# fegennari/3DWorld

Hardware: NVIDIA H100
Metric: height cells/s @8192^2 8-octave domain-warp (higher is better)
Workload: dtype f32

## Files before the change

3dworld_b200/csrc/tw_heightgen.cu:

```cuda
#include "tw_internal.h"
#include <unordered_map>
#include <vector>
#include <algorithm>
#include "tw_noise.cuh"
#include "tw_noise2.cuh"
#include <stdlib.h>

namespace {

constexpr int F_TABLE = TW_F_TABLE_SIZE;

__device__ __forceinline__ float sinf_lut(const float *__restrict__ tab, float v) {
	return (v < 0.0f) ? -__ldg(tab + (tw_x86_f2i(TW_SSCALE*(-v))&(TW_TSIZE-1))) : __ldg(tab + (tw_x86_f2i(TW_SSCALE*v)&(TW_TSIZE-1)));
}
__device__ __forceinline__ float cosf_lut(const float *__restrict__ tab, float v) {
	return __ldg(tab + TW_TSIZE + (tw_x86_f2i(TW_SSCALE*fabsf(v))&(TW_TSIZE-1)));
}
__device__ __forceinline__ float smin(float a, float b) {return (b < a) ? b : a;}
__device__ __forceinline__ float smax(float a, float b) {return (a < b) ? b : a;}

struct PostParams {
	tw_hmap_params h;
	int   shape;
	int   need_postproc;
	int   enable_glaciate;
	int   glaciate;
	float zmax_est, zmax_est2, zmax_est2_inv, custom_exp;
	int   sine_on;
	float sm_scale, sm_freq, sine_offset;
	int   volcano_on;
	float volcano_freq;
	float mesh_scale_z_inv;
	float mdx, mdy, dx_inv, dy_inv;
	const unsigned *tile_perm;
	unsigned ngroups;
	unsigned skip_x0, skip_y0, skip_w, skip_h;
};

__device__ __forceinline__ float postproc_noise_zval(float z, const tw_hmap_params &h) {
	if (z > h.plat_bot) {z = h.plat_bot + h.plat_h*(z - h.plat_bot) + smin(h.plat_max, h.plat_s*(z - h.plat_bot));}
	if (z > h.crat_h  ) {z = h.crat_h - h.crat_s*(z - h.crat_h);}
	if (z > h.crack_lo && z < h.crack_hi) {z -= h.crack_d*smin(z - h.crack_lo, h.crack_hi - z);}
	return z;
}

__device__ __forceinline__ float volcano_height(float xi, float yi, const PostParams &P, const float *__restrict__ tab) {
	float const x = P.volcano_freq*xi, y = P.volcano_freq*yi, dist = __fsqrt_rn(x*x + y*y);
	if ((double)dist > 2.0) return 0.0f;
	float const val = cosf_lut(tab, x)*cosf_lut(tab, y);
	double const hd = 400.0*((double)val - 0.999);
	float const hole = (float)((0.0 < hd) ? hd : 0.0);
	float const peak = (float)(0.08*(double)val/(double)smax(0.04f, dist));
	return P.h.volcano_height*smax(0.0f, (peak - hole))*P.mesh_scale_z_inv;
}

__device__ __forceinline__ float glaciate_and_bias(float z, float smx, float smy, float cx, float cy, const PostParams &P, const float *__restrict__ tab) {
	if (!P.enable_glaciate) return z;
	if (P.glaciate) {
		float const relh = (z + P.zmax_est)*P.zmax_est2_inv;
		float const g = (P.custom_exp == 0.0f) ? relh*relh*relh : powf(relh, P.custom_exp);
		z = g*P.zmax_est2 - P.zmax_est;
	}
	if (P.sine_on) {
		z += smx*smy + P.sine_offset;
		if (P.volcano_on) {z += volcano_height(cx, cy, P, tab);}
	}
	return z;
}

__device__ __forceinline__ void block_minmax(float vmin, float vmax, unsigned *mm) {
	for (int o = 16; o > 0; o >>= 1) {
		vmin = fminf(vmin, __shfl_xor_sync(0xffffffffu, vmin, o));
		vmax = fmaxf(vmax, __shfl_xor_sync(0xffffffffu, vmax, o));
	}
	__shared__ float s_min[32], s_max[32];
	int const tid = threadIdx.x + blockDim.x*(threadIdx.y + blockDim.y*threadIdx.z);
	int const nw = (blockDim.x*blockDim.y*blockDim.z + 31) >> 5, w = tid >> 5, l = tid & 31;
	if (l == 0) {s_min[w] = vmin; s_max[w] = vmax;}
	__syncthreads();
	if (w == 0) {
		vmin = (l < nw) ? s_min[l] :  INFINITY;
		vmax = (l < nw) ? s_max[l] : -INFINITY;
		for (int o = 16; o > 0; o >>= 1) {
			vmin = fminf(vmin, __shfl_xor_sync(0xffffffffu, vmin, o));
			vmax = fmaxf(vmax, __shfl_xor_sync(0xffffffffu, vmax, o));
		}
		if (l == 0) {atomicMin(mm, tw_f2ord(vmin)); atomicMax(mm + 1, tw_f2ord(vmax));}
	}
}

struct NoiseParams {
	int   octaves;
	int   gen_shape;
	float4 oct[9];
	float xy_scale;
	float hmap_scale;
	float freq_last, rsum_last;
};

template<bool SIMPLEX, int SHAPE>
__device__ __forceinline__ float gen_noise(float xv, float yv, const NoiseParams &N) {
	float zval = 0.0f;
#pragma unroll 1
	for (int i = 0; i < N.octaves; ++i) {
		float4 const o = N.oct[i];
		float const px = o.x*xv + o.y, py = o.x*yv + o.z;
		float noise = SIMPLEX ? twn::simplex2(px, py) : twn::perlin2(px, py);
		if (SHAPE == 1) {noise = (float)((double)fabsf(noise) - 0.40);}
		if (SHAPE == 2) {noise = (float)(0.45 - (double)fabsf(noise));}
		zval = __fmaf_rn(o.w, noise, zval);
	}
	return zval;
}

template<bool SIMPLEX, bool WARP, int SHAPE>
__device__ __forceinline__ float get_noise_zval(float xval, float yval, const NoiseParams &N, const PostParams &P) {
	float xv = N.xy_scale*xval, yv = N.xy_scale*yval;
	if (WARP) {
		float const scale = 0.2f;
		float const dx1 = gen_noise<SIMPLEX, SHAPE>((float)((double)xv + 0.0), (float)((double)yv + 0.0), N);
		float const dy1 = gen_noise<SIMPLEX, SHAPE>((float)((double)xv + 5.2), (float)((double)yv + 1.3), N);
		float const wx = xv + scale*dx1, wy = yv + scale*dy1;
		float const dx2 = gen_noise<SIMPLEX, SHAPE>((float)((double)wx + 1.7), (float)((double)wy + 9.2), N);
		float const dy2 = gen_noise<SIMPLEX, SHAPE>((float)((double)wx + 8.3), (float)((double)wy + 2.8), N);
		xv += scale*dx2; yv += scale*dy2;
	}
	float z = gen_noise<SIMPLEX, SHAPE>(xv, yv, N);
	if (P.need_postproc) {z = postproc_noise_zval(z, P.h);}
	return z*N.hmap_scale;
}

template<bool SIMPLEX, bool WARP, int SHAPE>
__global__ void __launch_bounds__(256)
noise_grid_kernel(float *__restrict__ out, unsigned nx, unsigned ny, unsigned y_off, float mx0_single, float my0_single, const float2 *__restrict__ tile_origins,
	NoiseParams N, PostParams P, const float *__restrict__ sin_tab, unsigned *__restrict__ mm)
{
	unsigned const x = blockIdx.x*blockDim.x + threadIdx.x, y = y_off + blockIdx.y*blockDim.y + threadIdx.y, tile = blockIdx.z;
	float mx0 = mx0_single, my0 = my0_single;
	if (tile_origins) {float2 const o = __ldg(tile_origins + tile); mx0 = o.x; my0 = o.y;}
	float z = 0.0f;
	bool const valid = (x < nx && y < ny);
	if (valid) {
		float const xval = ((float)x*P.mdx + mx0)*P.dx_inv, yval = ((float)y*P.mdy + my0)*P.dy_inv;
		z = get_noise_zval<SIMPLEX, WARP, SHAPE>(xval, yval, N, P);
		float smx = 0.0f, smy = 0.0f;
		if (P.enable_glaciate && P.sine_on) {
			smx = P.sm_scale*cosf_lut(sin_tab, ((float)x*P.mdx + mx0)*P.dx_inv*P.sm_freq);
			smy = cosf_lut(sin_tab, ((float)y*P.mdy + my0)*P.dy_inv*P.sm_freq);
		}
		z = glaciate_and_bias(z, smx, smy, xval, yval, P, sin_tab);
		out[(size_t)tile*nx*ny + (size_t)y*nx + x] = z;
	}
	if (mm) {block_minmax(valid ? z : INFINITY, valid ? z : -INFINITY, mm + 2*tile);}
}

#ifndef TW_NOISE2_MIN_BLOCKS
#define TW_NOISE2_MIN_BLOCKS 2
#endif
#ifndef TW_NOISE2_PERSISTENT
#define TW_NOISE2_PERSISTENT 1
#endif
#ifndef TW_NOISE2_THREADS
#define TW_NOISE2_THREADS 512
#endif
#ifndef TW_NOISE2_BLOCK_CELLS
#define TW_NOISE2_BLOCK_CELLS 2048
#endif
static_assert(TW_NOISE2_BLOCK_CELLS % (2*TW_NOISE2_THREADS) == 0, "a block walks whole chunks of 2 cells per thread");
__device__ __forceinline__ bool noise_lattice_in_range(float2 xv, float2 yv, const NoiseParams &N) {
	float const bx = (fabsf(xv.x) + fabsf(yv.x))*N.freq_last + N.rsum_last, by = (fabsf(xv.y) + fabsf(yv.y))*N.freq_last + N.rsum_last;
	return (bx < 2097152.0f && by < 2097152.0f);
}

template<bool SIMPLEX, bool WARP> __host__ __device__ constexpr bool noise2_hash() {return SIMPLEX && WARP && TW_SIMPLEX_HASH_TABLE;}
template<bool HASH> __host__ __device__ constexpr int lut_entries() {return twn2::SIMPLEX_LUT_N + (HASH ? twn2::SIMPLEX_HASH_N : 0);}
template<bool HASH> __host__ __device__ constexpr int lut_slots() {return twn2::SIMPLEX_LUT_N*twn2::SIMPLEX_LUT_COPIES + (HASH ? twn2::SIMPLEX_HASH_N*twn2::SIMPLEX_HASH_COPIES : 0);}

template<bool SIMPLEX, int SHAPE, bool HASH>
__device__ __forceinline__ float2 noise2_octave(float2 xv, float2 yv, float4 o, unsigned L, float2 zval) {
	float2 const px = twn2::add2(twn2::mul2(xv, o.x), o.y), py = twn2::add2(twn2::mul2(yv, o.x), o.z);
	float2 noise = SIMPLEX ? ((TW_SIMPLEX_LUT > 0) ? twn2::simplex2_lut<HASH>(px, py, L) : twn2::simplex2(px, py)) : ((TW_SIMPLEX_LUT > 0) ? twn2::perlin2_lut(px, py, L) : twn2::perlin2(px, py));
	if (SHAPE == 1) {noise = make_float2((float)((double)fabsf(noise.x) - 0.40), (float)((double)fabsf(noise.y) - 0.40));}
	if (SHAPE == 2) {noise = make_float2((float)(0.45 - (double)fabsf(noise.x)), (float)(0.45 - (double)fabsf(noise.y)));}
	return twn2::fma2(noise, o.w, zval);
}

template<bool SIMPLEX, int SHAPE, bool HASH>
__device__ __forceinline__ float2 gen_noise2(float2 xv, float2 yv, const NoiseParams &N, unsigned L) {
	float2 zval = make_float2(0.0f, 0.0f);
	bool const in_range = noise_lattice_in_range(xv, yv, N);
	if (HASH && SHAPE == 0 && N.octaves == 8 && in_range) {
#pragma unroll
		for (int i = 0; i < 8; ++i) {zval = noise2_octave<SIMPLEX, SHAPE, HASH>(xv, yv, N.oct[i], L, zval);}
	}
	else if (in_range) {
#pragma unroll 1
		for (int i = 0; i < N.octaves; ++i) {zval = noise2_octave<SIMPLEX, SHAPE, HASH>(xv, yv, N.oct[i], L, zval);}
	}
	else {zval = make_float2(gen_noise<SIMPLEX, SHAPE>(xv.x, yv.x, N), gen_noise<SIMPLEX, SHAPE>(xv.y, yv.y, N));}
	return zval;
}

#ifndef TW_NOISE2_DUAL
#define TW_NOISE2_DUAL 0
#endif
template<bool SIMPLEX, int SHAPE, bool HASH>
__device__ __forceinline__ void gen_noise2_dual(float2 xa, float2 ya, float2 xb, float2 yb, const NoiseParams &N, unsigned L, float2 &za, float2 &zb) {
	if (TW_SIMPLEX_LUT > 0 && noise_lattice_in_range(xa, ya, N) && noise_lattice_in_range(xb, yb, N)) {
		float2 zva = make_float2(0.0f, 0.0f), zvb = make_float2(0.0f, 0.0f);
#pragma unroll 1
		for (int i = 0; i < N.octaves; ++i) {
			float4 const o = N.oct[i];
			float const f = o.x, rx = o.y, ry = o.z, mag = o.w;
			float2 const pxa = twn2::add2(twn2::mul2(xa, f), rx), pya = twn2::add2(twn2::mul2(ya, f), ry);
			float2 const pxb = twn2::add2(twn2::mul2(xb, f), rx), pyb = twn2::add2(twn2::mul2(yb, f), ry);
			float2 na = SIMPLEX ? twn2::simplex2_lut<HASH>(pxa, pya, L) : twn2::perlin2_lut(pxa, pya, L);
			float2 nb = SIMPLEX ? twn2::simplex2_lut<HASH>(pxb, pyb, L) : twn2::perlin2_lut(pxb, pyb, L);
			if (SHAPE == 1) {na = make_float2((float)((double)fabsf(na.x) - 0.40), (float)((double)fabsf(na.y) - 0.40)); nb = make_float2((float)((double)fabsf(nb.x) - 0.40), (float)((double)fabsf(nb.y) - 0.40));}
			if (SHAPE == 2) {na = make_float2((float)(0.45 - (double)fabsf(na.x)), (float)(0.45 - (double)fabsf(na.y))); nb = make_float2((float)(0.45 - (double)fabsf(nb.x)), (float)(0.45 - (double)fabsf(nb.y)));}
			zva = twn2::fma2(na, mag, zva); zvb = twn2::fma2(nb, mag, zvb);
		}
		za = zva; zb = zvb;
	}
	else {za = gen_noise2<SIMPLEX, SHAPE, HASH>(xa, ya, N, L); zb = gen_noise2<SIMPLEX, SHAPE, HASH>(xb, yb, N, L);}
}

__device__ __forceinline__ float dadd(float a, double b) {return (float)((double)a + b);}
__constant__ double2 warp_offsets[4] = {{0.0, 0.0}, {5.2, 1.3}, {1.7, 9.2}, {8.3, 2.8}};

template<bool SIMPLEX, bool WARP, int SHAPE>
__global__ void __launch_bounds__(TW_NOISE2_THREADS, TW_NOISE2_MIN_BLOCKS)
noise_grid2_kernel(float *__restrict__ out, unsigned nx, unsigned ny, unsigned y_off, unsigned y_end, float mx0_single, float my0_single, const float2 *__restrict__ tile_origins,
	NoiseParams N, PostParams P, const float *__restrict__ sin_tab, unsigned *__restrict__ mm, const float4 *__restrict__ simplex_lut)
{
	constexpr bool HASH = noise2_hash<SIMPLEX, WARP>();
	unsigned L = 0;
	if (TW_SIMPLEX_LUT > 0) {
		extern __shared__ float4 lut_s[];
		constexpr int G = twn2::SIMPLEX_LUT_N*twn2::SIMPLEX_LUT_COPIES;
		for (int e = threadIdx.x; e < lut_slots<HASH>(); e += blockDim.x) {
			lut_s[e] = __ldg(simplex_lut + ((e < G) ? e/twn2::SIMPLEX_LUT_COPIES : twn2::SIMPLEX_LUT_N + (e - G)/twn2::SIMPLEX_HASH_COPIES));
		}
		__syncthreads();
		L = twn2::simplex_lut_base(lut_s, threadIdx.x);
		asm volatile("" : "+r"(L) :: "memory");
	}
	unsigned const tile = blockIdx.z;
	float mx0 = mx0_single, my0 = my0_single;
	if (tile_origins) {float2 const o = __ldg(tile_origins + tile); mx0 = o.x; my0 = o.y;}
	size_t const c_end = (size_t)y_end*nx;
	float lo = INFINITY, hi = -INFINITY;
	constexpr unsigned NCH = TW_NOISE2_BLOCK_CELLS/(2*TW_NOISE2_THREADS);
#pragma unroll 1
	for (unsigned grp = blockIdx.x; grp < P.ngroups; grp += gridDim.x) {
#pragma unroll 1
	for (unsigned ch = 0; ch < NCH; ++ch) {
	size_t const c0 = (size_t)y_off*nx + 2*(((size_t)grp*NCH + ch)*blockDim.x + threadIdx.x);
	unsigned y, x;
	if (c_end <= 0xffffffffull) {unsigned const c32 = (unsigned)c0; y = c32/nx; x = c32 - y*nx;}
	else {y = (unsigned)(c0/nx); x = (unsigned)(c0 - (size_t)y*nx);}
	unsigned const xb = (x + 1 < nx) ? x + 1 : 0, yb = (x + 1 < nx) ? y : y + 1;
	bool const skip = (x - P.skip_x0 < P.skip_w && y - P.skip_y0 < P.skip_h && xb - P.skip_x0 < P.skip_w && yb - P.skip_y0 < P.skip_h);
	bool const valid0 = (c0 < c_end) && !skip, valid1 = (c0 + 1 < c_end) && !skip;
	float z0 = 0.0f, z1 = 0.0f;
	if (valid0) {
		using namespace twn2;
		float2 const xs = make_float2((float)x, (float)xb), ys = make_float2((float)y, (float)yb);
		float2 const xval = mul2(add2(mul2(xs, P.mdx), mx0), P.dx_inv);
		float2 const yval = mul2(add2(mul2(ys, P.mdy), my0), P.dy_inv);
		float2 xv = mul2(xval, N.xy_scale), yv = mul2(yval, N.xy_scale);
		float2 zz;
		if (WARP && !TW_NOISE2_DUAL) {
			float const scale = 0.2f;
			float2 bx = xv, by = yv, d = make_float2(0.0f, 0.0f);
#pragma unroll 1
			for (int s = 0; s < 5; ++s) {
				float2 sx = xv, sy = yv;
				if (s < 4) {double2 const o = warp_offsets[s]; sx = make_float2(dadd(bx.x, o.x), dadd(bx.y, o.x)); sy = make_float2(dadd(by.x, o.y), dadd(by.y, o.y));}
				float2 const r = gen_noise2<SIMPLEX, SHAPE, HASH>(sx, sy, N, L);
				if (s == 1) {bx = add2(xv, mul2(d, scale)); by = add2(yv, mul2(r, scale));}
				if (s == 3) {xv = add2(xv, mul2(d, scale)); yv = add2(yv, mul2(r, scale));}
				d = r;
			}
			zz = d;
		}
		else {
		if (WARP) {
			float const scale = 0.2f;
			float2 dx1, dy1, dx2, dy2;
			gen_noise2_dual<SIMPLEX, SHAPE, HASH>(make_float2(dadd(xv.x, 0.0), dadd(xv.y, 0.0)), make_float2(dadd(yv.x, 0.0), dadd(yv.y, 0.0)),
			                                      make_float2(dadd(xv.x, 5.2), dadd(xv.y, 5.2)), make_float2(dadd(yv.x, 1.3), dadd(yv.y, 1.3)), N, L, dx1, dy1);
			float2 const wx = add2(xv, mul2(dx1, scale)), wy = add2(yv, mul2(dy1, scale));
			gen_noise2_dual<SIMPLEX, SHAPE, HASH>(make_float2(dadd(wx.x, 1.7), dadd(wx.y, 1.7)), make_float2(dadd(wy.x, 9.2), dadd(wy.y, 9.2)),
			                                      make_float2(dadd(wx.x, 8.3), dadd(wx.y, 8.3)), make_float2(dadd(wy.x, 2.8), dadd(wy.y, 2.8)), N, L, dx2, dy2);
			xv = add2(xv, mul2(dx2, scale)); yv = add2(yv, mul2(dy2, scale));
		}
		zz = gen_noise2<SIMPLEX, SHAPE, HASH>(xv, yv, N, L);
		}
		z0 = zz.x; z1 = zz.y;
		if (P.need_postproc) {z0 = postproc_noise_zval(z0, P.h); z1 = postproc_noise_zval(z1, P.h);}
		z0 = z0*N.hmap_scale; z1 = z1*N.hmap_scale;
		float smx0 = 0.0f, smx1 = 0.0f, smy0 = 0.0f, smy1 = 0.0f;
		if (P.enable_glaciate && P.sine_on) {
			smx0 = P.sm_scale*cosf_lut(sin_tab, xval.x*P.sm_freq);
			smx1 = P.sm_scale*cosf_lut(sin_tab, xval.y*P.sm_freq);
			smy0 = cosf_lut(sin_tab, yval.x*P.sm_freq);
			smy1 = (yb == y) ? smy0 : cosf_lut(sin_tab, yval.y*P.sm_freq);
		}
		z0 = glaciate_and_bias(z0, smx0, smy0, xval.x, yval.x, P, sin_tab);
		z1 = glaciate_and_bias(z1, smx1, smy1, xval.y, yval.y, P, sin_tab);
		float *o = out + (size_t)(P.tile_perm ? __ldg(P.tile_perm + tile) : tile)*nx*ny + c0;
		if (valid1 && ((reinterpret_cast<size_t>(o) & 7) == 0)) {*reinterpret_cast<float2 *>(o) = make_float2(z0, z1);}
		else {o[0] = z0; if (valid1) {o[1] = z1;}}
	}
	lo = fminf(lo, fminf(valid0 ? z0 : INFINITY, valid1 ? z1 : INFINITY)); hi = fmaxf(hi, fmaxf(valid0 ? z0 : -INFINITY, valid1 ? z1 : -INFINITY));
	}
	}
	if (mm) {block_minmax(lo, hi, mm + 2*tile);}
}

template<bool SIMPLEX, bool WARP>
void launch_noise2(int shape, dim3 grid, dim3 block, cudaStream_t st, float *out, unsigned nx, unsigned ny, unsigned y_off, unsigned y_end, float mx0, float my0,
	const float2 *origins, const NoiseParams &N, const PostParams &P, const float *tab, unsigned *mm, const float4 *lut)
{
	size_t const lut_bytes = (TW_SIMPLEX_LUT > 0) ? (size_t)lut_slots<noise2_hash<SIMPLEX, WARP>()>()*sizeof(float4) : 0;
	if (lut_bytes > 48*1024) {
		switch (shape) {
		case 1:  cudaFuncSetAttribute(noise_grid2_kernel<SIMPLEX, WARP, 1>, cudaFuncAttributeMaxDynamicSharedMemorySize, (int)lut_bytes); break;
		case 2:  cudaFuncSetAttribute(noise_grid2_kernel<SIMPLEX, WARP, 2>, cudaFuncAttributeMaxDynamicSharedMemorySize, (int)lut_bytes); break;
		default: cudaFuncSetAttribute(noise_grid2_kernel<SIMPLEX, WARP, 0>, cudaFuncAttributeMaxDynamicSharedMemorySize, (int)lut_bytes); break;
		}
	}
	switch (shape) {
	case 1:  noise_grid2_kernel<SIMPLEX, WARP, 1><<<grid, block, lut_bytes, st>>>(out, nx, ny, y_off, y_end, mx0, my0, origins, N, P, tab, mm, lut); break;
	case 2:  noise_grid2_kernel<SIMPLEX, WARP, 2><<<grid, block, lut_bytes, st>>>(out, nx, ny, y_off, y_end, mx0, my0, origins, N, P, tab, mm, lut); break;
	default: noise_grid2_kernel<SIMPLEX, WARP, 0><<<grid, block, lut_bytes, st>>>(out, nx, ny, y_off, y_end, mx0, my0, origins, N, P, tab, mm, lut); break;
	}
}

constexpr int PERLIN_LUT_OFFSET = lut_entries<true>();
__global__ void simplex_lut_kernel(float4 *__restrict__ lut) {
	int const k = blockIdx.x*blockDim.x + threadIdx.x;
	if (k < twn2::SIMPLEX_LUT_N) {lut[k] = twn2::simplex_lut_entry((float)k); lut[PERLIN_LUT_OFFSET + k] = twn2::perlin_lut_entry((float)k);}
	if (k < twn2::SIMPLEX_HASH_N) {lut[twn2::SIMPLEX_LUT_N + k] = twn2::simplex_hash_entry((float)k);}
}
static int ensure_simplex_lut(tw_ctx *ctx) {
	if (ctx->d_simplex_lut) return TW_OK;
	static_assert(twn2::SIMPLEX_HASH_N <= twn2::SIMPLEX_LUT_N, "simplex_lut_kernel's grid covers the gradient tables");
	TW_CUDA(ctx, cudaMalloc(&ctx->d_simplex_lut, (PERLIN_LUT_OFFSET + twn2::SIMPLEX_LUT_N)*sizeof(float4)));
	simplex_lut_kernel<<<(twn2::SIMPLEX_LUT_N + 127)/128, 128, 0, ctx->stream>>>((float4 *)ctx->d_simplex_lut);
	TW_LAUNCH_CHECK(ctx);
	return TW_OK;
}

struct SineTabParams {
	float msx, msy, ms2, mesh_scale_z_inv;
	float dx, dy, mx0, my0;
	int   start;
	unsigned nx, ny, xpitch, ypitch;
	int   sine_on; float sm_scale, sm_freq, dx_inv, dy_inv;
};

__global__ void sine_tables_kernel(float *__restrict__ Xt, float *__restrict__ Yt, const float *__restrict__ T, const float *__restrict__ sin_tab, SineTabParams S,
	const float *__restrict__ origins = nullptr, unsigned nux = 0, size_t xstride = 0, size_t ystride = 0)
{
	unsigned const i = blockIdx.x*blockDim.x + threadIdx.x, k = blockIdx.y;
	bool const is_y = origins ? (blockIdx.z >= nux) : (blockIdx.z != 0);
	if (origins) {
		if (is_y) {S.my0 = __ldg(origins + blockIdx.z); Yt += (size_t)(blockIdx.z - nux)*ystride;}
		else      {S.mx0 = __ldg(origins + blockIdx.z); Xt += (size_t)blockIdx.z*xstride;}
	}
	unsigned const n = is_y ? S.ny : S.nx;
	if (i >= n) return;
	if (k == F_TABLE) {
		if (!S.sine_on) return;
		if (!is_y) {Xt[(size_t)k*S.xpitch + i] = S.sm_scale*cosf_lut(sin_tab, ((float)i*S.dx + S.mx0)*S.dx_inv*S.sm_freq);}
		else       {Yt[(size_t)k*S.ypitch + i] = cosf_lut(sin_tab, ((float)i*S.dy + S.my0)*S.dy_inv*S.sm_freq);}
		return;
	}
	if ((int)k < S.start) return;
	float const *s = T + 5*k;
	if (!is_y) {
		float const x_mult = S.msx*s[4];
		float const x_const = S.ms2*s[4] + s[2] + x_mult*S.mx0;
		float const xmdx = x_mult*S.dx;
		Xt[(size_t)k*S.xpitch + i] = sinf_lut(sin_tab, xmdx*(float)i + x_const);
	}
	else {
		float const y_mult = S.msy*s[3], y_scale = S.mesh_scale_z_inv*s[0];
		float const y_const = S.ms2*s[3] + s[1] + y_mult*S.my0;
		float const ymdy = y_mult*S.dy;
		Yt[(size_t)k*S.ypitch + i] = y_scale*sinf_lut(sin_tab, ymdy*(float)i + y_const);
	}
}

constexpr int ST = 64;
constexpr int SK = 45;

__global__ void __launch_bounds__(256)
sine_grid_kernel(float *__restrict__ out, unsigned nx, unsigned ny, const float *__restrict__ Xt, const float *__restrict__ Yt,
	unsigned xpitch, unsigned ypitch, int start_ix, PostParams P, float mx0, float my0, const float *__restrict__ sin_tab, unsigned *__restrict__ mm, unsigned y_off,
	const uint2 *__restrict__ tile_tabs = nullptr, const float2 *__restrict__ tile_origins = nullptr, size_t xstride = 0, size_t ystride = 0,
	const unsigned *__restrict__ tile_perm = nullptr)
{
	__shared__ float Xs[SK][ST], Ys[SK][ST];
	if (tile_tabs) {
		unsigned const tz = tile_perm ? __ldg(tile_perm + blockIdx.z) : blockIdx.z;
		uint2 const tt = __ldg(tile_tabs + tz);
		float2 const o = __ldg(tile_origins + tz);
		Xt += (size_t)tt.x*xstride; Yt += (size_t)tt.y*ystride; mx0 = o.x; my0 = o.y;
		out += (size_t)blockIdx.z*nx*ny;
		if (mm) {mm += 2*(size_t)blockIdx.z;}
	}
	unsigned const x_base = blockIdx.x*ST, y_base = y_off + blockIdx.y*ST;
	int const tid = threadIdx.x, tx = tid & 15, ty = tid >> 4;
	float2 acc2[4][2];
#pragma unroll
	for (int a = 0; a < 4; ++a) {acc2[a][0] = make_float2(0.0f, 0.0f); acc2[a][1] = make_float2(0.0f, 0.0f);}
	for (int k0 = start_ix; k0 < F_TABLE; k0 += SK) {
		int const kn = min(SK, F_TABLE - k0);
		__syncthreads();
		for (int e = tid; e < kn*ST; e += 256) {
			int const kk = e / ST, c = e % ST;
			unsigned const gx = x_base + c, gy = y_base + c;
			Xs[kk][c] = (gx < nx) ? __ldg(Xt + (size_t)(k0 + kk)*xpitch + gx) : 0.0f;
			Ys[kk][c] = (gy < ny) ? __ldg(Yt + (size_t)(k0 + kk)*ypitch + gy) : 0.0f;
		}
		__syncthreads();
#pragma unroll 5
		for (int kk = 0; kk < kn; ++kk) {
			float xv[4];
#pragma unroll
			for (int b = 0; b < 4; ++b) {xv[b] = Xs[kk][tx + 16*b];}
			float4 const yv4 = *reinterpret_cast<const float4 *>(&Ys[kk][ty*4]);
			float const yv[4] = {yv4.x, yv4.y, yv4.z, yv4.w};
			float2 const x01 = make_float2(xv[0], xv[1]), x23 = make_float2(xv[2], xv[3]);
#pragma unroll
			for (int a = 0; a < 4; ++a) {
				float2 const ya = twn2::splat(yv[a]);
				acc2[a][0] = twn2::add2(twn2::mul2(x01, ya), acc2[a][0]);
				acc2[a][1] = twn2::add2(twn2::mul2(x23, ya), acc2[a][1]);
			}
		}
	}
	float vmin = INFINITY, vmax = -INFINITY;
#pragma unroll
	for (int a = 0; a < 4; ++a) {
		unsigned const y = y_base + ty*4 + a;
		if (y >= ny) continue;
		float const smy = (P.enable_glaciate && P.sine_on) ? __ldg(Yt + (size_t)F_TABLE*ypitch + y) : 0.0f;
#pragma unroll
		for (int b = 0; b < 4; ++b) {
			unsigned const x = x_base + tx + 16*b;
			if (x >= nx) continue;
			float z = (b & 1) ? ((b >> 1) ? acc2[a][1].y : acc2[a][0].y) : ((b >> 1) ? acc2[a][1].x : acc2[a][0].x);
			if (P.shape == 1) {z = (float)((double)fabsf(z) - 2.0);}
			else if (P.shape == 2) {z = (float)(3.5 - (double)fabsf(z));}
			if (P.need_postproc) {z = postproc_noise_zval(z, P.h);}
			float const smx = (P.enable_glaciate && P.sine_on) ? __ldg(Xt + (size_t)F_TABLE*xpitch + x) : 0.0f;
			float cx = 0.0f, cy = 0.0f;
			if (P.volcano_on) {cx = ((float)x*P.mdx + mx0)*P.dx_inv; cy = ((float)y*P.mdy + my0)*P.dy_inv;}
			z = glaciate_and_bias(z, smx, smy, cx, cy, P, sin_tab);
			out[(size_t)y*nx + x] = z;
			vmin = fminf(vmin, z); vmax = fmaxf(vmax, z);
		}
	}
	if (mm) {block_minmax(vmin, vmax, mm);}
}

__global__ void init_minmax_kernel(unsigned *mm, uint32_t n) {
	uint32_t const i = blockIdx.x*blockDim.x + threadIdx.x;
	if (i < n) {mm[2*i] = 0xffffffffu; mm[2*i+1] = 0u;}
}

__global__ void minmax_kernel(const float *__restrict__ v, size_t n, unsigned *mm) {
	float vmin = INFINITY, vmax = -INFINITY;
	size_t const stride = (size_t)gridDim.x*blockDim.x;
	for (size_t i = (size_t)blockIdx.x*blockDim.x + threadIdx.x; i < n; i += stride) {float const z = __ldg(v + i); vmin = fminf(vmin, z); vmax = fmaxf(vmax, z);}
	block_minmax(vmin, vmax, mm);
}

__global__ void minmax_tiles_kernel(const float *__restrict__ v, size_t tile_elems, unsigned *mm, const unsigned *__restrict__ perm) {
	size_t const tile = perm ? __ldg(perm + blockIdx.x) : blockIdx.x;
	const float *t = v + tile*tile_elems;
	if (threadIdx.x == 0) {mm[2*tile] = 0xffffffffu; mm[2*tile + 1] = 0u;}
	__syncthreads();
	float vmin = INFINITY, vmax = -INFINITY;
	for (size_t i = threadIdx.x; i < tile_elems; i += blockDim.x) {float const z = __ldg(t + i); vmin = fminf(vmin, z); vmax = fmaxf(vmax, z);}
	block_minmax(vmin, vmax, mm + 2*tile);
}
__global__ void coarse_work_kernel(const float *__restrict__ coarse, unsigned cells, unsigned nt, float level, unsigned *__restrict__ work) {
	unsigned const t = blockIdx.x*blockDim.x + threadIdx.x;
	if (t >= nt) return;
	unsigned n = 0;
	for (unsigned i = 0; i < cells; ++i) {n += !(__ldg(coarse + (size_t)t*cells + i) < level);}
	work[t] = n;
}
__global__ void gather_origins_kernel(const float2 *__restrict__ org, const unsigned *__restrict__ order, unsigned nt, float2 *__restrict__ out) {
	unsigned const t = blockIdx.x*blockDim.x + threadIdx.x;
	if (t < nt) {out[t] = org[order[t]];}
}

template<bool SIMPLEX, bool WARP>
void launch_noise(int shape, dim3 grid, dim3 block, cudaStream_t st, float *out, unsigned nx, unsigned ny, unsigned y_off, float mx0, float my0,
	const float2 *origins, const NoiseParams &N, const PostParams &P, const float *tab, unsigned *mm)
{
	switch (shape) {
	case 1:  noise_grid_kernel<SIMPLEX, WARP, 1><<<grid, block, 0, st>>>(out, nx, ny, y_off, mx0, my0, origins, N, P, tab, mm); break;
	case 2:  noise_grid_kernel<SIMPLEX, WARP, 2><<<grid, block, 0, st>>>(out, nx, ny, y_off, mx0, my0, origins, N, P, tab, mm); break;
	default: noise_grid_kernel<SIMPLEX, WARP, 0><<<grid, block, 0, st>>>(out, nx, ny, y_off, mx0, my0, origins, N, P, tab, mm); break;
	}
}

}

int twi_init_minmax(tw_ctx *ctx, unsigned *d_mm_ord, uint32_t n) {
	init_minmax_kernel<<<(n + 255)/256, 256, 0, ctx->stream>>>(d_mm_ord, n);
	TW_LAUNCH_CHECK(ctx);
	return TW_OK;
}

int twi_minmax_tiles(tw_ctx *ctx, cudaStream_t st, const float *d_vals, size_t tile_elems, uint32_t nt, unsigned *d_mm_ord, const unsigned *d_perm) {
	minmax_tiles_kernel<<<nt, 256, 0, st>>>(d_vals, tile_elems, d_mm_ord, d_perm);
	TW_LAUNCH_CHECK(ctx);
	return TW_OK;
}
int twi_coarse_work(tw_ctx *ctx, const float *d_coarse, unsigned cells, uint32_t nt, float level, unsigned *d_work) {
	coarse_work_kernel<<<(nt + 127)/128, 128, 0, ctx->stream>>>(d_coarse, cells, nt, level, d_work);
	TW_LAUNCH_CHECK(ctx);
	return TW_OK;
}
int twi_gather_origins(tw_ctx *ctx, const void *d_org, const unsigned *d_order, uint32_t nt, void *d_out) {
	gather_origins_kernel<<<(nt + 255)/256, 256, 0, ctx->stream>>>((const float2 *)d_org, d_order, nt, (float2 *)d_out);
	TW_LAUNCH_CHECK(ctx);
	return TW_OK;
}

int twi_minmax(tw_ctx *ctx, const float *d_vals, size_t n, unsigned *d_mm_ord) {
	int const blocks = (int)((n + 255)/256 < ctx->num_sms*8 ? (n + 255)/256 : ctx->num_sms*8);
	minmax_kernel<<<blocks > 0 ? blocks : 1, 256, 0, ctx->stream>>>(d_vals, n, d_mm_ord);
	TW_LAUNCH_CHECK(ctx);
	return TW_OK;
}

static unsigned band_rows_for(tw_ctx *ctx, unsigned ny, unsigned nx, bool to_host) {
	if (!to_host || (size_t)nx*ny*sizeof(float) < ((size_t)32 << 20) || !ctx->aux_stream[0]) return ny;
	unsigned rows = ((ny + 15)/16 + 63) & ~63u;
	return rows < 64 ? 64 : rows;
}
static int band_join(tw_ctx *ctx) {
	cudaEvent_t ev;
	TW_CUDA(ctx, cudaEventCreateWithFlags(&ev, cudaEventDisableTiming));
	TW_CUDA(ctx, cudaEventRecord(ev, ctx->aux_stream[0]));
	TW_CUDA(ctx, cudaStreamWaitEvent(ctx->stream, ev, 0));
	TW_CUDA(ctx, cudaEventDestroy(ev));
	return TW_OK;
}

static int band_copy(tw_ctx *ctx, float *h_out, const float *d_out, unsigned nx, unsigned r0, unsigned r1) {
	cudaEvent_t ev;
	TW_CUDA(ctx, cudaEventCreateWithFlags(&ev, cudaEventDisableTiming));
	TW_CUDA(ctx, cudaEventRecord(ev, ctx->stream));
	TW_CUDA(ctx, cudaStreamWaitEvent(ctx->aux_stream[0], ev, 0));
	TW_CUDA(ctx, cudaEventDestroy(ev));
	TW_CUDA(ctx, cudaMemcpyAsync(h_out + (size_t)r0*nx, d_out + (size_t)r0*nx, (size_t)(r1 - r0)*nx*sizeof(float), cudaMemcpyDeviceToHost, ctx->aux_stream[0]));
	return TW_OK;
}

static PostParams make_post_params(const tw_height_params *p, int enable_glaciate, float dx, float dy) {
	PostParams P;
	memset(&P, 0, sizeof(P));
	P.h = p->hmap;
	P.shape = p->gen_shape;
	P.need_postproc = 1;
	P.enable_glaciate = (enable_glaciate != 0);
	P.glaciate = (p->glaciate != 0);
	P.zmax_est = p->zmax_est;
	P.zmax_est2 = (float)(2.0*p->zmax_est);
	P.zmax_est2_inv = (float)(1.0/P.zmax_est2);
	P.custom_exp = p->custom_glaciate_exp;
	P.sine_on = (p->hmap.sine_mag > 0.0f);
	P.sm_scale = p->hmap.sine_mag*p->mesh_scale_z_inv;
	P.sm_freq = p->mesh_scale*p->hmap.sine_freq;
	P.sine_offset = p->hmap.sine_bias*p->mesh_scale_z_inv;
	P.volcano_on = (p->hmap.volcano_width > 0.0f && p->hmap.volcano_height > 0.0f);
	P.volcano_freq = P.volcano_on ? p->mesh_scale/p->hmap.volcano_width : 0.0f;
	P.mesh_scale_z_inv = p->mesh_scale_z_inv;
	P.mdx = dx; P.mdy = dy; P.dx_inv = p->dx_val_inv; P.dy_inv = p->dy_val_inv;
	return P;
}

static bool make_noise_params(const tw_height_params *p, NoiseParams &N, bool &simplex) {
	memset(&N, 0, sizeof(N));
	int const start = p->start_eval_sin;
	if (start < 0 || start > F_TABLE) return false;
	N.octaves = 9 - start/10;
	N.gen_shape = p->gen_shape;
	float mag = 1.0f, freq = 1.0f, rx = p->rx, ry = p->ry;
	for (int i = 0; i < 9; ++i) {
		N.oct[i] = make_float4(freq, rx, ry, mag);
		mag *= 0.5f; freq *= 1.92f; rx *= 1.5f; ry *= 1.5f;
	}
	float4 const last = N.oct[N.octaves > 0 ? N.octaves - 1 : 0];
	N.freq_last = last.x; N.rsum_last = last.y + last.z;
	N.xy_scale = 0.0007f*p->mesh_scale;
	simplex = (p->gen_mode == TW_MGEN_SIMPLEX || p->gen_mode == TW_MGEN_SIMPLEX_GPU || p->gen_mode == TW_MGEN_DWARP_GPU);
	N.hmap_scale = (simplex ? 16.0f : 32.0f)*p->mesh_height*p->mesh_height_scale*p->mesh_scale_z_inv;
	return true;
}

int twi_heightgen(tw_ctx *ctx, const tw_grid2d *g, const tw_height_params *p, int enable_glaciate, int min_start_sin,
                  const float2 *d_tile_origins, uint32_t ntiles, float *d_out, unsigned *d_mm_ord, float *h_out_bands)
{
	unsigned const nx = g->nx, ny = g->ny;
	float const dx = g->dx, dy = g->dy;
	float const mx0 = dx*g->x0, my0 = dy*g->y0;
	if (ntiles == 0) ntiles = 1;

	PostParams P = make_post_params(p, enable_glaciate, dx, dy);
	P.skip_x0 = ctx->skip_rect[0]; P.skip_y0 = ctx->skip_rect[1]; P.skip_w = ctx->skip_rect[2]; P.skip_h = ctx->skip_rect[3];
	P.tile_perm = ctx->tile_perm;
	if (P.tile_perm && (p->gen_mode == TW_MGEN_SINE || getenv("TW_NOISE_SCALAR"))) return tw_set_error(ctx, TW_ERR_STATE, "internal: tile_perm is only wired into the paired noise kernels");

	if (p->gen_mode != TW_MGEN_SINE) {
		NoiseParams N;
		bool simplex = false;
		if (!make_noise_params(p, N, simplex)) return tw_set_error(ctx, TW_ERR_ARG, "start_eval_sin %d out of range", p->start_eval_sin);
		bool const warp = (p->gen_mode == TW_MGEN_DWARP_GPU);
		{int const rc = ensure_simplex_lut(ctx); if (rc) return rc;}
		const float4 *lut = (const float4 *)ctx->d_simplex_lut + (simplex ? 0 : PERLIN_LUT_OFFSET);
		unsigned const band_rows = band_rows_for(ctx, ny, nx, h_out_bands != nullptr && ntiles == 1);
		for (unsigned r0 = 0; r0 < ny; r0 += band_rows) {
			unsigned const r1 = (ny - r0 < band_rows) ? ny : r0 + band_rows;
			static bool const use_scalar = (getenv("TW_NOISE_SCALAR") != nullptr);
			if (!use_scalar) {
				size_t const band_cells = (size_t)(r1 - r0)*nx;
				unsigned gx = (unsigned)((band_cells + TW_NOISE2_BLOCK_CELLS - 1)/TW_NOISE2_BLOCK_CELLS);
				P.ngroups = gx;
#if TW_NOISE2_PERSISTENT
				{unsigned const wave = ctx->num_sms*TW_NOISE2_MIN_BLOCKS*TW_NOISE2_PERSISTENT; if (ntiles == 1 && gx > wave) gx = wave;}
#endif
				dim3 const block(TW_NOISE2_THREADS, 1, 1), grid(gx, 1, ntiles);
				if (p->gen_mode == TW_MGEN_PERLIN) {launch_noise2<false, false>(p->gen_shape, grid, block, ctx->stream, d_out, nx, ny, r0, r1, mx0, my0, d_tile_origins, N, P, ctx->d_sin_table, d_mm_ord, lut);}
				else if (warp) {launch_noise2<true, true >(p->gen_shape, grid, block, ctx->stream, d_out, nx, ny, r0, r1, mx0, my0, d_tile_origins, N, P, ctx->d_sin_table, d_mm_ord, lut);}
				else           {launch_noise2<true, false>(p->gen_shape, grid, block, ctx->stream, d_out, nx, ny, r0, r1, mx0, my0, d_tile_origins, N, P, ctx->d_sin_table, d_mm_ord, lut);}
				TW_LAUNCH_CHECK(ctx);
				if (h_out_bands) {int const rc = band_copy(ctx, h_out_bands, d_out, nx, r0, r1); if (rc) return rc;}
				continue;
			}
			dim3 const block(32, 8, 1), grid((nx + 31)/32, (r1 - r0 + 7)/8, ntiles);
			if (p->gen_mode == TW_MGEN_PERLIN) {launch_noise<false, false>(p->gen_shape, grid, block, ctx->stream, d_out, nx, ny, r0, mx0, my0, d_tile_origins, N, P, ctx->d_sin_table, d_mm_ord);}
			else if (warp) {launch_noise<true, true >(p->gen_shape, grid, block, ctx->stream, d_out, nx, ny, r0, mx0, my0, d_tile_origins, N, P, ctx->d_sin_table, d_mm_ord);}
			else           {launch_noise<true, false>(p->gen_shape, grid, block, ctx->stream, d_out, nx, ny, r0, mx0, my0, d_tile_origins, N, P, ctx->d_sin_table, d_mm_ord);}
			TW_LAUNCH_CHECK(ctx);
			if (h_out_bands) {int const rc = band_copy(ctx, h_out_bands, d_out, nx, r0, r1); if (rc) return rc;}
		}
		return h_out_bands ? band_join(ctx) : TW_OK;
	}

	if (!ctx->have_sine_params) return tw_set_error(ctx, TW_ERR_STATE, "tw_set_sine_params() has not been called");
	if (d_tile_origins && ntiles > 1) return tw_set_error(ctx, TW_ERR_ARG, "internal: sine mode tiles are issued one grid at a time");
	unsigned const xpitch = (nx + 63) & ~63u, ypitch = (ny + 63) & ~63u;
	size_t const tab_floats = (size_t)(F_TABLE + 1)*(xpitch + ypitch);
	int rc = tw_reserve(ctx, 1, tab_floats*sizeof(float));
	if (rc) return rc;
	float *Xt = (float *)ctx->d_scratch[1], *Yt = Xt + (size_t)(F_TABLE + 1)*xpitch;
	SineTabParams S;
	memset(&S, 0, sizeof(S));
	S.msx = p->mesh_scale*p->dx_val_inv; S.msy = p->mesh_scale*p->dy_val_inv; S.ms2 = (float)(0.5*p->mesh_scale);
	S.mesh_scale_z_inv = p->mesh_scale_z_inv;
	S.dx = dx; S.dy = dy; S.mx0 = mx0; S.my0 = my0;
	S.start = p->start_eval_sin;
	S.nx = nx; S.ny = ny; S.xpitch = xpitch; S.ypitch = ypitch;
	S.sine_on = (enable_glaciate && p->hmap.sine_mag != 0.0f); S.sm_scale = P.sm_scale; S.sm_freq = P.sm_freq; S.dx_inv = p->dx_val_inv; S.dy_inv = p->dy_val_inv;
	{
		unsigned const nmax = nx > ny ? nx : ny;
		dim3 const grid((nmax + 255)/256, F_TABLE + 1, 2);
		sine_tables_kernel<<<grid, 256, 0, ctx->stream>>>(Xt, Yt, ctx->d_sine_params, ctx->d_sin_table, S);
		TW_LAUNCH_CHECK(ctx);
	}
	int const start_ix = (p->start_eval_sin > min_start_sin) ? p->start_eval_sin : min_start_sin;
	unsigned const band_rows = band_rows_for(ctx, ny, nx, h_out_bands != nullptr);
	for (unsigned r0 = 0; r0 < ny; r0 += band_rows) {
		unsigned const r1 = (ny - r0 < band_rows) ? ny : r0 + band_rows;
		dim3 const grid((nx + ST - 1)/ST, (r1 - r0 + ST - 1)/ST, 1);
		sine_grid_kernel<<<grid, 256, 0, ctx->stream>>>(d_out, nx, ny, Xt, Yt, xpitch, ypitch, start_ix, P, mx0, my0, ctx->d_sin_table, d_mm_ord, r0);
		TW_LAUNCH_CHECK(ctx);
		if (h_out_bands) {int const rc = band_copy(ctx, h_out_bands, d_out, nx, r0, r1); if (rc) return rc;}
	}
	return h_out_bands ? band_join(ctx) : TW_OK;
}

size_t twi_sine_tiles_stage_bytes(uint32_t ntiles) {return (size_t)ntiles*(2*sizeof(float) + sizeof(uint2) + sizeof(float2));}

namespace {
struct SineTilesLayout {size_t tab_bytes, org_bytes, tt_bytes, to_bytes;};
SineTilesLayout sine_tiles_layout(const tw_grid2d *g, size_t nux, size_t nuy, uint32_t ntiles) {
	size_t const xstride = (size_t)(F_TABLE + 1)*((g->nx + 63) & ~63u), ystride = (size_t)(F_TABLE + 1)*((g->ny + 63) & ~63u);
	return SineTilesLayout{((nux*xstride + nuy*ystride)*sizeof(float) + 255) & ~(size_t)255, ((nux + nuy)*sizeof(float) + 255) & ~(size_t)255,
	                       ((size_t)ntiles*sizeof(uint2) + 255) & ~(size_t)255, ((size_t)ntiles*sizeof(float2) + 255) & ~(size_t)255};
}
}

size_t twi_sine_tiles_plan(const tw_grid2d *g, const float2 *h_org, uint32_t ntiles, twi_sine_batch *b) {
	std::unordered_map<uint32_t, unsigned> mx, my;
	std::vector<float> uy;
	b->uorg.clear(); b->tabs.resize(ntiles);
	for (uint32_t t = 0; t < ntiles; ++t) {
		uint32_t bx, by;
		memcpy(&bx, &h_org[t].x, 4); memcpy(&by, &h_org[t].y, 4);
		auto ix = mx.find(bx); if (ix == mx.end()) {ix = mx.emplace(bx, (unsigned)b->uorg.size()).first; b->uorg.push_back(h_org[t].x);}
		auto iy = my.find(by); if (iy == my.end()) {iy = my.emplace(by, (unsigned)uy.size()).first; uy.push_back(h_org[t].y);}
		b->tabs[t] = make_uint2(ix->second, iy->second);
	}
	b->nux = (unsigned)b->uorg.size(); b->nuy = (unsigned)uy.size();
	b->uorg.insert(b->uorg.end(), uy.begin(), uy.end());
	SineTilesLayout const L = sine_tiles_layout(g, b->nux, b->nuy, ntiles);
	return L.tab_bytes + L.org_bytes + L.tt_bytes + L.to_bytes;
}

int twi_sine_tiles_setup(tw_ctx *ctx, const tw_grid2d *g, const tw_height_params *p, int enable_glaciate, int min_start_sin, const float2 *h_org, uint32_t ntiles,
                         void *d_mem, void *h_stage, twi_sine_batch *b)
{
	if (!ctx->have_sine_params) return tw_set_error(ctx, TW_ERR_STATE, "tw_set_sine_params() has not been called");
	unsigned const nx = g->nx, ny = g->ny;
	PostParams const P = make_post_params(p, enable_glaciate, g->dx, g->dy);
	unsigned const nux = b->nux, nuy = b->nuy;
	if (nux + nuy > 65535) return tw_set_error(ctx, TW_ERR_ARG, "more than 65535 distinct tile rows + columns in one batch");
	unsigned const xpitch = (nx + 63) & ~63u, ypitch = (ny + 63) & ~63u;
	size_t const xstride = (size_t)(F_TABLE + 1)*xpitch, ystride = (size_t)(F_TABLE + 1)*ypitch;
	SineTilesLayout const L = sine_tiles_layout(g, nux, nuy, ntiles);
	if (!d_mem) {
		int const rc = tw_reserve(ctx, 1, L.tab_bytes + L.org_bytes + L.tt_bytes + L.to_bytes);
		if (rc) return rc;
		d_mem = ctx->d_scratch[1];
	}
	char *sp = (char *)d_mem;
	float *Xt = (float *)sp, *Yt = Xt + nux*xstride; sp += L.tab_bytes;
	float *d_uorg = (float *)sp; sp += L.org_bytes;
	uint2 *d_tabs = (uint2 *)sp; sp += L.tt_bytes;
	float2 *d_torg = (float2 *)sp;
	std::vector<float> const &uorg = b->uorg;
	const void *src_uorg = uorg.data(), *src_tabs = b->tabs.data(), *src_org = h_org;
	if (h_stage) {
		char *hs = (char *)h_stage;
		memcpy(hs, uorg.data(), uorg.size()*sizeof(float)); src_uorg = hs; hs += (size_t)2*ntiles*sizeof(float);
		memcpy(hs, b->tabs.data(), (size_t)ntiles*sizeof(uint2)); src_tabs = hs; hs += (size_t)ntiles*sizeof(uint2);
		memcpy(hs, h_org, (size_t)ntiles*sizeof(float2)); src_org = hs;
	}
	TW_CUDA(ctx, cudaMemcpyAsync(d_uorg, src_uorg, uorg.size()*sizeof(float), cudaMemcpyHostToDevice, ctx->stream));
	TW_CUDA(ctx, cudaMemcpyAsync(d_tabs, src_tabs, (size_t)ntiles*sizeof(uint2), cudaMemcpyHostToDevice, ctx->stream));
	TW_CUDA(ctx, cudaMemcpyAsync(d_torg, src_org, (size_t)ntiles*sizeof(float2), cudaMemcpyHostToDevice, ctx->stream));
	SineTabParams S;
	memset(&S, 0, sizeof(S));
	S.msx = p->mesh_scale*p->dx_val_inv; S.msy = p->mesh_scale*p->dy_val_inv; S.ms2 = (float)(0.5*p->mesh_scale);
	S.mesh_scale_z_inv = p->mesh_scale_z_inv;
	S.dx = g->dx; S.dy = g->dy;
	S.start = p->start_eval_sin;
	S.nx = nx; S.ny = ny; S.xpitch = xpitch; S.ypitch = ypitch;
	S.sine_on = (enable_glaciate && p->hmap.sine_mag != 0.0f); S.sm_scale = P.sm_scale; S.sm_freq = P.sm_freq; S.dx_inv = p->dx_val_inv; S.dy_inv = p->dy_val_inv;
	unsigned const nmax = nx > ny ? nx : ny;
	sine_tables_kernel<<<dim3((nmax + 255)/256, F_TABLE + 1, nux + nuy), 256, 0, ctx->stream>>>(Xt, Yt, ctx->d_sine_params, ctx->d_sin_table, S, d_uorg, nux, xstride, ystride);
	TW_LAUNCH_CHECK(ctx);
	if (!h_stage) {TW_CUDA(ctx, cudaStreamSynchronize(ctx->stream));}
	b->g = *g; b->p = *p; b->enable_glaciate = enable_glaciate; b->min_start_sin = min_start_sin;
	b->Xt = Xt; b->Yt = Yt; b->d_tabs = d_tabs; b->d_torg = d_torg; b->xstride = xstride; b->ystride = ystride; b->xpitch = xpitch; b->ypitch = ypitch;
	return TW_OK;
}

int twi_sine_tiles_grid(tw_ctx *ctx, const twi_sine_batch *b, uint32_t t0, uint32_t nt, const unsigned *d_perm, float *d_out, unsigned *d_mm_ord) {
	unsigned const nx = b->g.nx, ny = b->g.ny;
	PostParams const P = make_post_params(&b->p, b->enable_glaciate, b->g.dx, b->g.dy);
	int const start_ix = (b->p.start_eval_sin > b->min_start_sin) ? b->p.start_eval_sin : b->min_start_sin;
	for (uint32_t c0 = 0; c0 < nt; c0 += 65535) {
		uint32_t const cn = std::min<uint32_t>(65535u, nt - c0);
		size_t const s = (size_t)t0 + c0;
		sine_grid_kernel<<<dim3((nx + ST - 1)/ST, (ny + ST - 1)/ST, cn), 256, 0, ctx->stream>>>(d_out + (size_t)c0*nx*ny, nx, ny, b->Xt, b->Yt, b->xpitch, b->ypitch, start_ix, P, 0.0f, 0.0f,
			ctx->d_sin_table, d_mm_ord ? d_mm_ord + 2*(size_t)c0 : nullptr, 0, d_perm ? b->d_tabs : b->d_tabs + s, d_perm ? b->d_torg : b->d_torg + s, b->xstride, b->ystride,
			d_perm ? d_perm + s : nullptr);
		TW_LAUNCH_CHECK(ctx);
	}
	return TW_OK;
}

int twi_heightgen_sine_tiles(tw_ctx *ctx, const tw_grid2d *g, const tw_height_params *p, int enable_glaciate, int min_start_sin, const float2 *h_org, uint32_t ntiles,
                             float *d_out, unsigned *d_mm_ord, void *h_stage)
{
	twi_sine_batch b;
	twi_sine_tiles_plan(g, h_org, ntiles, &b);
	int rc = twi_sine_tiles_setup(ctx, g, p, enable_glaciate, min_start_sin, h_org, ntiles, nullptr, h_stage, &b); if (rc) return rc;
	return twi_sine_tiles_grid(ctx, &b, 0, ntiles, nullptr, d_out, d_mm_ord);
// ... 99 lines not shown
```

Before: 8.756 billion.

## Restructure domain-warp stages and chunk scheduling with incremental cell indexing

Replaces the strided group/chunk loop with contiguous per-block chunk ranges whose (x,y) position is advanced incrementally, so the per-chunk 64-bit division is gone. The domain-warp stage loop is rewritten to precompute shifted coordinates. A single hoisted range check lets the fully unrolled 8-octave path, which reads split per-component octave arrays, be used for all five warp stages instead of re-checking each stage. The skip-rectangle test is also bypassed when no skip is set. It adds a conservative shift bound for the range check, and the new incremental indexing and chunk split carry correctness risk.

```diff
diff --git a/3dworld_b200/csrc/tw_heightgen.cu b/3dworld_b200/csrc/tw_heightgen.cu
--- a/3dworld_b200/csrc/tw_heightgen.cu
+++ b/3dworld_b200/csrc/tw_heightgen.cu
@@ -33,7 +33,8 @@
 	float mesh_scale_z_inv;
 	float mdx, mdy, dx_inv, dy_inv;
 	const unsigned *tile_perm;
-	unsigned ngroups;
+	unsigned nchunks;
+	unsigned step_q, step_r;
 	unsigned skip_x0, skip_y0, skip_w, skip_h;
 };
 
@@ -93,6 +94,7 @@
 	int   octaves;
 	int   gen_shape;
 	float4 oct[9];
+	float freq8[8], rx8[8], ry8[8], mag8[8];
 	float xy_scale;
 	float hmap_scale;
 	float freq_last, rsum_last;
@@ -185,15 +187,25 @@
 	return twn2::fma2(noise, o.w, zval);
 }
 
+template<bool HASH>
+__device__ __forceinline__ float2 gen_noise2_8(float2 xv, float2 yv, const NoiseParams &N, unsigned L) {
+	float2 zval = make_float2(0.0f, 0.0f);
+#pragma unroll
+	for (int i = 0; i < 8; ++i) {zval = noise2_octave<true, 0, HASH>(xv, yv, make_float4(N.freq8[i], N.rx8[i], N.ry8[i], N.mag8[i]), L, zval);}
+	return zval;
+}
+
+constexpr float DWARP_MAX_SHIFT = 20.0f;
+__device__ __forceinline__ bool dwarp_lattice_in_range(float2 xv, float2 yv, const NoiseParams &N) {
+	float const bx = ((fabsf(xv.x) + fabsf(yv.x)) + 2.0f*DWARP_MAX_SHIFT)*N.freq_last + N.rsum_last;
+	float const by = ((fabsf(xv.y) + fabsf(yv.y)) + 2.0f*DWARP_MAX_SHIFT)*N.freq_last + N.rsum_last;
+	return (bx < 2097152.0f && by < 2097152.0f);
+}
+
 template<bool SIMPLEX, int SHAPE, bool HASH>
 __device__ __forceinline__ float2 gen_noise2(float2 xv, float2 yv, const NoiseParams &N, unsigned L) {
 	float2 zval = make_float2(0.0f, 0.0f);
-	bool const in_range = noise_lattice_in_range(xv, yv, N);
-	if (HASH && SHAPE == 0 && N.octaves == 8 && in_range) {
-#pragma unroll
-		for (int i = 0; i < 8; ++i) {zval = noise2_octave<SIMPLEX, SHAPE, HASH>(xv, yv, N.oct[i], L, zval);}
-	}
-	else if (in_range) {
+	if (noise_lattice_in_range(xv, yv, N)) {
 #pragma unroll 1
 		for (int i = 0; i < N.octaves; ++i) {zval = noise2_octave<SIMPLEX, SHAPE, HASH>(xv, yv, N.oct[i], L, zval);}
 	}
@@ -226,8 +238,27 @@
 }
 
 __device__ __forceinline__ float dadd(float a, double b) {return (float)((double)a + b);}
-__constant__ double2 warp_offsets[4] = {{0.0, 0.0}, {5.2, 1.3}, {1.7, 9.2}, {8.3, 2.8}};
-
+__device__ __forceinline__ float2 dadd2(float2 a, double b) {return make_float2(dadd(a.x, b), dadd(a.y, b));}
+
+template<class FBM>
+__device__ __forceinline__ float2 dwarp_stages(float2 xv, float2 yv, FBM fbm) {
+	using namespace twn2;
+	float const scale = 0.2f;
+	float2 sx = add2(xv, 0.0f), sy = add2(yv, 0.0f), tx = dadd2(xv, 5.2), ty = dadd2(yv, 1.3), d = make_float2(0.0f, 0.0f);
+	bool odd = false;
+#pragma unroll 1
+	for (int s = 0; s < 5; ++s) {
+		float2 const r = fbm(sx, sy);
+		if (!odd) {d = r; sx = tx; sy = ty;}
+		else if (s == 1) {
+			float2 const wx = add2(xv, mul2(d, scale)), wy = add2(yv, mul2(r, scale));
+			sx = dadd2(wx, 1.7); sy = dadd2(wy, 9.2); tx = dadd2(wx, 8.3); ty = dadd2(wy, 2.8);
+		}
+		else {sx = add2(xv, mul2(d, scale)); sy = add2(yv, mul2(r, scale));}
+		odd = !odd;
+	}
+	return d;
+}
 template<bool SIMPLEX, bool WARP, int SHAPE>
 __global__ void __launch_bounds__(TW_NOISE2_THREADS, TW_NOISE2_MIN_BLOCKS)
 noise_grid2_kernel(float *__restrict__ out, unsigned nx, unsigned ny, unsigned y_off, unsigned y_end, float mx0_single, float my0_single, const float2 *__restrict__ tile_origins,
@@ -248,20 +279,21 @@
 	unsigned const tile = blockIdx.z;
 	float mx0 = mx0_single, my0 = my0_single;
 	if (tile_origins) {float2 const o = __ldg(tile_origins + tile); mx0 = o.x; my0 = o.y;}
-	size_t const c_end = (size_t)y_end*nx;
 	float lo = INFINITY, hi = -INFINITY;
-	constexpr unsigned NCH = TW_NOISE2_BLOCK_CELLS/(2*TW_NOISE2_THREADS);
+	unsigned const k0 = (unsigned)((size_t)P.nchunks*blockIdx.x/gridDim.x), k1 = (unsigned)((size_t)P.nchunks*(blockIdx.x + 1)/gridDim.x);
+	unsigned y, x;
+	{
+		size_t const c = (size_t)y_off*nx + 2*((size_t)k0*blockDim.x + threadIdx.x);
+		if (c <= 0xffffffffull) {unsigned const c32 = (unsigned)c; y = c32/nx; x = c32 - y*nx;}
+		else {y = (unsigned)(c/nx); x = (unsigned)(c - (size_t)y*nx);}
+	}
 #pragma unroll 1
-	for (unsigned grp = blockIdx.x; grp < P.ngroups; grp += gridDim.x) {
-#pragma unroll 1
-	for (unsigned ch = 0; ch < NCH; ++ch) {
-	size_t const c0 = (size_t)y_off*nx + 2*(((size_t)grp*NCH + ch)*blockDim.x + threadIdx.x);
-	unsigned y, x;
-	if (c_end <= 0xffffffffull) {unsigned const c32 = (unsigned)c0; y = c32/nx; x = c32 - y*nx;}
-	else {y = (unsigned)(c0/nx); x = (unsigned)(c0 - (size_t)y*nx);}
+	for (unsigned k = k0; k < k1; ++k) {
 	unsigned const xb = (x + 1 < nx) ? x + 1 : 0, yb = (x + 1 < nx) ? y : y + 1;
-	bool const skip = (x - P.skip_x0 < P.skip_w && y - P.skip_y0 < P.skip_h && xb - P.skip_x0 < P.skip_w && yb - P.skip_y0 < P.skip_h);
-	bool const valid0 = (c0 < c_end) && !skip, valid1 = (c0 + 1 < c_end) && !skip;
+	bool skip = false;
+	if (P.skip_w != 0) {skip = (x - P.skip_x0 < P.skip_w && y - P.skip_y0 < P.skip_h && xb - P.skip_x0 < P.skip_w && yb - P.skip_y0 < P.skip_h);}
+	bool const valid0 = (y < y_end) && !skip, valid1 = (yb < y_end) && !skip;
+	size_t const c0 = (size_t)y*nx + x;
 	float z0 = 0.0f, z1 = 0.0f;
 	if (valid0) {
 		using namespace twn2;
@@ -271,18 +303,8 @@
 		float2 xv = mul2(xval, N.xy_scale), yv = mul2(yval, N.xy_scale);
 		float2 zz;
 		if (WARP && !TW_NOISE2_DUAL) {
-			float const scale = 0.2f;
-			float2 bx = xv, by = yv, d = make_float2(0.0f, 0.0f);
-#pragma unroll 1
-			for (int s = 0; s < 5; ++s) {
-				float2 sx = xv, sy = yv;
-				if (s < 4) {double2 const o = warp_offsets[s]; sx = make_float2(dadd(bx.x, o.x), dadd(bx.y, o.x)); sy = make_float2(dadd(by.x, o.y), dadd(by.y, o.y));}
-				float2 const r = gen_noise2<SIMPLEX, SHAPE, HASH>(sx, sy, N, L);
-				if (s == 1) {bx = add2(xv, mul2(d, scale)); by = add2(yv, mul2(r, scale));}
-				if (s == 3) {xv = add2(xv, mul2(d, scale)); yv = add2(yv, mul2(r, scale));}
-				d = r;
-			}
-			zz = d;
+			if (HASH && SHAPE == 0 && N.octaves == 8 && dwarp_lattice_in_range(xv, yv, N)) {zz = dwarp_stages(xv, yv, [&](float2 x, float2 y) {return gen_noise2_8<HASH>(x, y, N, L);});}
+			else {zz = dwarp_stages(xv, yv, [&](float2 x, float2 y) {return gen_noise2<SIMPLEX, SHAPE, HASH>(x, y, N, L);});}
 		}
 		else {
 		if (WARP) {
@@ -314,7 +336,7 @@
 		else {o[0] = z0; if (valid1) {o[1] = z1;}}
 	}
 	lo = fminf(lo, fminf(valid0 ? z0 : INFINITY, valid1 ? z1 : INFINITY)); hi = fmaxf(hi, fmaxf(valid0 ? z0 : -INFINITY, valid1 ? z1 : -INFINITY));
-	}
+	if (x >= nx - P.step_r) {x -= nx - P.step_r; y += P.step_q + 1;} else {x += P.step_r; y += P.step_q;}
 	}
 	if (mm) {block_minmax(lo, hi, mm + 2*tile);}
 }
@@ -599,6 +621,7 @@
 	float mag = 1.0f, freq = 1.0f, rx = p->rx, ry = p->ry;
 	for (int i = 0; i < 9; ++i) {
 		N.oct[i] = make_float4(freq, rx, ry, mag);
+		if (i < 8) {N.freq8[i] = freq; N.rx8[i] = rx; N.ry8[i] = ry; N.mag8[i] = mag;}
 		mag *= 0.5f; freq *= 1.92f; rx *= 1.5f; ry *= 1.5f;
 	}
 	float4 const last = N.oct[N.octaves > 0 ? N.octaves - 1 : 0];
@@ -636,7 +659,9 @@
 			if (!use_scalar) {
 				size_t const band_cells = (size_t)(r1 - r0)*nx;
 				unsigned gx = (unsigned)((band_cells + TW_NOISE2_BLOCK_CELLS - 1)/TW_NOISE2_BLOCK_CELLS);
-				P.ngroups = gx;
+				size_t const chunk = 2*TW_NOISE2_THREADS;
+				P.nchunks = (unsigned)((band_cells + chunk - 1)/chunk);
+				P.step_q = (unsigned)(chunk/nx); P.step_r = (unsigned)(chunk%nx);
 #if TW_NOISE2_PERSISTENT
 				{unsigned const wave = ctx->num_sms*TW_NOISE2_MIN_BLOCKS*TW_NOISE2_PERSISTENT; if (ntiles == 1 && gx > wave) gx = wave;}
 #endif
```

Result: faster. 8.971 billion (median of 6 runs) (+2.5%).
